# althonos/pyopal

Measured on AMD Instinct MI355X. Metric: GCUPS (billion DP cells/s) SW score-only, 53aa query vs 1Mx300aa DB, higher is better.
Workload: dtype u16; 1 GPU; sw_score q53 (README.md:86) vs 1000000x300 uniform-random proteins per GPU, BLOSUM62, gap_open 3, gap_extend 1; value: blocking miopalSearch, scores in the caller's pinned host array (value_device_results: scores left in HBM); targets_per_gpu=1000000, target_length=300, query_length=53

## Files before the change

include/miopal.h:

```cpp
#ifndef MIOPAL_H
#define MIOPAL_H

#include <stdint.h>

#include "opal.h"

#ifdef __cplusplus
extern "C" {
#endif

typedef struct MiopalDb MiopalDb;

int miopalDeviceCount(void);

const char* miopalLastError(void);

int miopalDbCreate(MiopalDb** out, const unsigned char* const* sequences, const int* lengths,
                   int64_t count, int alphabetLength, int device);

int miopalDbCreateFlat(MiopalDb** out, const unsigned char* residues, const int64_t* offsets,
                       int64_t count, int alphabetLength, int device);

int miopalDbCreateSubset(MiopalDb** out, const MiopalDb* parent, const int64_t* indices, int64_t count);

// ... 23 lines not shown
                         int gapExt, const int* scoreMatrix, int alphabetLength, int searchType,
                         int mode, int64_t start, int64_t end, int* score, int* endTarget,
                         int* endQuery, int* startTarget, int* startQuery,
                         unsigned char** operations, int64_t* operationsCapacity,
                         int64_t* operationOffsets);

int miopalSearchDeviceScores(MiopalDb* db, const unsigned char* query, int queryLength,
                             int gapOpen, int gapExt, const int* scoreMatrix,
                             int alphabetLength, int mode, int64_t start, int64_t end,
                             int* deviceScores, void* stream);

void miopalSetProfiling(MiopalDb* db, int enabled);
int miopalLastKernelTime(MiopalDb* db, float* ms);

void miopalLastRouting(int64_t counts[4]);

int miopalSearchBatch(MiopalDb* db, const unsigned char* queries, const int64_t* queryOffsets, int nQueries,
                      int gapOpen, int gapExt, const int* scoreMatrix, int alphabetLength, int searchType,
                      int mode, int64_t start, int64_t end, int* score, int* endTarget, int* endQuery);

#define MIOPAL_MAX_TOP 4096
int miopalSearchTop(MiopalDb* db, const unsigned char* query, int queryLength, int gapOpen, int gapExt,
                    const int* scoreMatrix, int alphabetLength, int searchType, int mode,
                    int64_t start, int64_t end, int k, int minScore,
                    int* count, int64_t* targetIndex, int* score, int* endTarget, int* endQuery);

int miopalSearchBatchTop(MiopalDb* db, const unsigned char* queries, const int64_t* queryOffsets, int nQueries,
                         int gapOpen, int gapExt, const int* scoreMatrix, int alphabetLength, int searchType,
                         int mode, int64_t start, int64_t end, int k, int minScore,
                         int* count, int64_t* targetIndex, int* score, int* endTarget, int* endQuery);
// ... 35 lines not shown
```

pyopal_amd/_capi.py:

```python

from __future__ import annotations

import ctypes
import os
import typing

import numpy as np

_HERE = os.path.dirname(os.path.abspath(__file__))
LIB_PATH = os.environ.get("MIOPAL_LIBRARY") or os.path.join(_HERE, "libmiopal.so")

OPAL_ERR_OVERFLOW = 1
OPAL_ERR_NO_SIMD_SUPPORT = 2
OPAL_ERR_INVALID_MODE = 3
MIOPAL_MAX_TOP = 4096

SEARCH = {"score": 0, "end": 1, "full": 2}
MODE = {"nw": 0, "hw": 1, "ov": 2, "sw": 3}
OVERFLOW = {"simple": 0, "buckets": 1}


class OpalSearchResult(ctypes.Structure):
    _fields_ = [
        ("scoreSet", ctypes.c_int),
# ... 4 lines not shown
        ("startLocationQuery", ctypes.c_int),
        ("alignment", ctypes.POINTER(ctypes.c_ubyte)),
        ("alignmentLength", ctypes.c_int),
    ]


_lib = None
_libc = None

EXPORTS = [
    "opalInitSearchResult", "opalSearchResultIsEmpty", "opalSearchResultSetScore",
    "opalSearchDatabase", "opalSearchDatabaseCharSW",
    "miopalDeviceCount", "miopalLastError", "miopalDbCreate", "miopalDbCreateFlat", "miopalDbCreateSubset",
    "miopalDbDestroy", "miopalDbCount", "miopalDbTotalLength", "miopalDbDeviceBytes",
    "miopalSearch", "miopalSearchFlat", "miopalSearchFlatInto", "miopalSearchDeviceScores", "miopalSetProfiling", "miopalLastKernelTime",
    "miopalLastRouting", "miopalLastFullRouting", "miopalSearchResults", "miopalReleaseCaches",
    "miopalSearchBatch", "miopalLastBatchRouting", "miopalSearchTop", "miopalSearchBatchTop",
    "miopalAlignPairs", "miopalLastPairRouting",
    "miopalSetTuning", "miopalGetTuning", "miopalDbSetOption", "miopalDbReleaseWorkspaces",
    "miopalSelfTest", "miopalTestInjectFault", "miopalTestSetLogicalDevices",
]


def _share_hip_runtime() -> None:
    import importlib.util
    try:
        spec = importlib.util.find_spec("torch")
    except (ImportError, ValueError):
        spec = None
    if spec is None or not spec.submodule_search_locations:
        return
# ... 64 lines not shown
                                       c_i64, c_i64, c_vp, c_vp, c_vp, c_vp, c_vp,
                                       ctypes.POINTER(c_vp), c_vp]
        L.miopalSearchFlatInto.restype = c_int
        L.miopalSearchFlatInto.argtypes = [c_vp, c_vp, c_int, c_int, c_int, c_vp, c_int, c_int, c_int,
                                           c_i64, c_i64, c_vp, c_vp, c_vp, c_vp, c_vp,
                                           ctypes.POINTER(c_vp), ctypes.POINTER(c_i64), c_vp]
        L.miopalSearchDeviceScores.restype = c_int
        L.miopalSearchDeviceScores.argtypes = [c_vp, c_vp, c_int, c_int, c_int, c_vp, c_int, c_int,
                                               c_i64, c_i64, c_vp, c_vp]
        L.miopalSetProfiling.restype = None
        L.miopalSetProfiling.argtypes = [c_vp, c_int]
        L.miopalReleaseCaches.restype = None
        L.miopalReleaseCaches.argtypes = []
        L.miopalLastFullRouting.restype = c_int
        L.miopalLastFullRouting.argtypes = []
        L.miopalLastRouting.restype = None
        L.miopalLastRouting.argtypes = [ctypes.POINTER(ctypes.c_int64)]
        L.miopalLastKernelTime.restype = c_int
        L.miopalLastKernelTime.argtypes = [c_vp, ctypes.POINTER(ctypes.c_float)]
        L.miopalSearchResults.restype = c_int
        L.miopalSearchResults.argtypes = [c_vp, c_vp, c_int, c_int, c_int, c_vp, c_int, c_vp, c_int,
                                          c_int, c_int, c_i64, c_i64]
        L.opalSearchDatabase.restype = c_int
        L.opalSearchDatabase.argtypes = [c_vp, c_int, c_vp, c_int, c_vp, c_int, c_int, c_vp, c_int,
                                         c_vp, c_int, c_int, c_int]
        _lib = L
        _libc = ctypes.CDLL(None)
        _libc.free.argtypes = [c_vp]
        _libc.free.restype = None
    return _lib
# ... 343 lines not shown
        end = self.count if end is None else min(end, self.count)
        q = np.ascontiguousarray(query, dtype=np.uint8)
        S = np.ascontiguousarray(matrix, dtype=np.int32)
        rc = lib().miopalSearchDeviceScores(self._h, _ptr(q), len(q), gap_open, gap_extend, _ptr(S),
                                            self.alphabet_length, MODE[algorithm], start, end,
                                            ctypes.c_void_p(device_ptr), ctypes.c_void_p(stream))
        raise_for(rc)

    @staticmethod
    def last_routing() -> typing.Tuple[int, int, int, int]:
        counts = (ctypes.c_int64 * 4)()
        lib().miopalLastRouting(counts)
        return tuple(int(c) for c in counts)

    @staticmethod
    def last_full_routing() -> int:
        return int(lib().miopalLastFullRouting())

    def set_profiling(self, enabled: bool) -> None:
        lib().miopalSetProfiling(self._h, 1 if enabled else 0)

    def last_kernel_time(self) -> typing.Tuple[int, float]:
        ms = ctypes.c_float(0)
        n = lib().miopalLastKernelTime(self._h, ctypes.byref(ms))
        return int(n), float(ms.value)
```

pyopal_amd/csrc/common.h:

```cpp
#pragma once
#include <hip/hip_runtime.h>
#include <stdint.h>

namespace miopal {

constexpr int kLanes = 64;
constexpr int kGroupTargets = 128;
constexpr int kMaxAlphabet = 32;
constexpr int kMaxStripRows = 64;

enum Region : int { kLastCell = 0, kLastRow = 1, kLastRowCol = 2, kAllCells = 3 };
struct DpRules {
    int topGap;
    int leftGap;
    int floor0;
    int region;
};

struct InterseqArgs {
    const uint2* pack;
    const int64_t* groupOff;
    const int* groupChunks;
    int nGroups;
    int groupBase;
// ... 22 lines not shown
    int tailThrottle;
    unsigned long long* stripKeys;
    int* stripAbort;
    int stripAbortAt;
    int* stripGaveUp;
    int batchGroups;
    const int32_t* known;
    int32_t* directOut;
    int32_t* directEndI;
    int32_t* directEndJ;
    const int32_t* directIds;
    int directN;
    int stripSpinCap;
    int faultUnit1;
    unsigned long long* stripTiming;
    uint2* boundary[2];
    const int64_t* boundaryOff;
};

struct BatchArgs {
    const uint2* pack;
    const int64_t* groupOff;
    const int* groupChunks;
    const int32_t* lens;
    const int32_t* ids;
    int nPacked;
    int64_t sliceStart;
    const int16_t* profiles;
    int nSymbols;
    const int* qLens;
    const int* qRows;
    int nQueries;
    int unitsPerQuery;
// ... 303 lines not shown
```

pyopal_amd/csrc/host.hip:

```cpp
#include <algorithm>
#include <atomic>
#include <chrono>
#include <condition_variable>
#if defined(__x86_64__)
#include <immintrin.h>
#endif
#include <cstdarg>
#include <cstdio>
#include <cstdlib>
#include <cstring>
#include <deque>
#include <functional>
#include <exception>
#include <ctime>
#include <list>
#include <map>
#include <memory>
#include <mutex>
#include <new>
#include <numeric>
#include <string>
#include <sys/mman.h>
#include <thread>
#include <vector>
// ... 31 lines not shown
        for (int k = 0; k < (int)Tune::kCount; ++k)
            if (strcmp(kTuningNames[k] + 7, name) == 0) return k;
        return -1;
    }
};
}
const char* tuned(Tune key) { return Tuning::table().value[(int)key].load(std::memory_order_acquire); }
}

namespace {

thread_local std::string g_lastError;
thread_local int64_t g_lastRouting[4] = {0, 0, 0, 0};
thread_local int64_t g_lastBatchRouting[4] = {0, 0, 0, 0};
thread_local int g_lastFullRouting = 0;
thread_local int g_fault[3] = {0, 0, 0};
std::atomic<int> g_logicalDevices{0};

const std::vector<int>& usableDevices() {
    static const std::vector<int> list = [] {
        std::vector<int> v;
        int n = 0;
        if (hipGetDeviceCount(&n) != hipSuccess) return v;
        for (int d = 0; d < n; ++d) {
            hipDeviceProp_t p;
            if (hipGetDeviceProperties(&p, d) == hipSuccess && strncmp(p.gcnArchName, "gfx950", 6) == 0) v.push_back(d);
        }
        return v;
    }();
    return list;
// ... 442 lines not shown
        waiter.join();
        if (rcWaiter != 0) return 4;
        if (db->views.size() != 1 || db->views.front().building) return 5;
        db->views.clear();
        return 0;
    });
}

void miopalLastRouting(int64_t counts[4]) {
    if (!counts) return;
    for (int k = 0; k < 4; ++k) counts[k] = g_lastRouting[k];
}

int miopalLastFullRouting(void) { return g_lastFullRouting; }

void miopalLastBatchRouting(int64_t counts[4]) {
    if (!counts) return;
    for (int k = 0; k < 4; ++k) counts[k] = g_lastBatchRouting[k];
}

int miopalLastKernelTime(MiopalDb* db, float* ms) {
    if (!db || !ms) return 0;
    std::lock_guard<std::mutex> g(db->timingMutex);
    *ms = 0.f;
    Workspace* ws = db->lastTimed;
    if (!ws) return 0;
    int n = 0;
    for (auto& ev : ws->timings) {
        float t = 0.f;
        if (hipEventSynchronize(ev.second) == hipSuccess &&
// ... 370 lines not shown
```

pyopal_amd/csrc/host_search.inc:

```
static inline int reservedCus(const MiopalDb* db) {
    const int opt = db->optReserveCus.load(std::memory_order_relaxed);
    if (opt >= 0) return opt;
    if (const char* r = tuned(Tune::RESERVE_CUS)) return std::max(0, atoi(r));
    return -1;
}
static inline bool smallSearchAllowed(const MiopalDb* db) {
    const int opt = db->optSmallSearch.load(std::memory_order_relaxed);
    if (opt >= 0) return opt != 0;
    return !tuned(Tune::NO_SMALL_SEARCH);
}

struct Search {
    MiopalDb* db;
    Workspace* ws;
    hipStream_t stream;
    const unsigned char* query;
    int Q, open, ext, A, searchType, mode;
    const int* matrix;
    int64_t start, end;
    int64_t n;
    int maxScore = 0, minScore = 0;
    int64_t balancedChunks = 0;
    bool globalPairRefused = false;
    bool pairStripsRefused = false;
// ... 190 lines not shown
    }

    int scorePass(int32_t* d_score, int32_t* d_endI, int32_t* d_endJ) {
        return scorePassImpl(d_score, d_endI, d_endJ, true);
    }

    int scorePassImpl(int32_t* d_score, int32_t* d_endI, int32_t* d_endJ, bool useHalf) {
        DpRules r;
        RC_TRY(rulesFor(mode, &r));
        const int rules = packRules(r);
        std::vector<PairJob> jobs;
        RC_TRY(checkInt32(db->maxLen));
        wroteHost = false;

        g_lastRouting[0] = g_lastRouting[1] = g_lastRouting[2] = g_lastRouting[3] = 0;
        bool small = Q <= kLanes && n <= kSmallSearch;
        if (Q > kLanes && n <= kSmallSearch) {
            const int64_t strips = ((int64_t)Q + kLanes - 1) / kLanes;
            const int64_t residues = db->offsets[(size_t)end] - db->offsets[(size_t)start];
            const int64_t steps = strips * (residues + (int64_t)(kLanes - 1) * n);
            if (const char* asked = tuned(Tune::SMALL_STEPS)) {
                small = steps <= atoll(asked);
            } else {
                const double perPair = 0.075 + std::max((double)steps / 7e6, (double)(db->maxLen + kLanes * strips) * 0.00025);
                const double packed = 0.26 + 0.0006 * (double)Q + (Q <= 512 ? 0.0003 * (double)db->maxLen : 0.0);
                small = perPair < packed;
            }
        }
        if (!interseqUsable() || (small && smallSearchAllowed(db))) {
            g_lastRouting[0] = n;
// ... 394 lines not shown
                sideForked = true;
                spt.mark("    side jobs enqueued");
                return 0;
            };
            if (!sideJobs.empty() && !tuned(Tune::NO_SIDE_STREAM)) {
                RC_TRY(ws->ensureAux());
                RC_TRY(ensurePairInputs());
                HIP_TRY(hipEventRecord(ws->evFork, stream));
                HIP_TRY(hipStreamWaitEvent(ws->aux, ws->evFork, 0));
                forked = true;
                sidePending = true;
                besidePersistent = pairStrips;
                if (!tuned(Tune::PACKED_FIRST)) RC_TRY(enqueueSide());
            }
            void *pp, *vs, *vo, *ct;
            RC_TRY(ws->get(kProfile, prof.size() * sizeof(int16_t), &pp));
            RC_TRY(ws->get(kViewScore, (size_t)view->nGroups * kGroupTargets * sizeof(int32_t), &vs));
            RC_TRY(ws->get(kViewOvf, (size_t)view->nGroups * kGroupTargets, &vo));
            RC_TRY(ws->get(kCounter, sizeof(int32_t), &ct));
            RC_TRY(ws->stageUpload(pp, prof.data(), prof.size() * sizeof(prof[0]), stream));
            const int64_t reach = std::min<int64_t>((int64_t)std::min(Q, view->maxPackedLen) * std::max(maxScore, 0), queryBest);
            const int64_t limit = (biased || pairStrips) ? biasedLimit : swShifted ? swLimit : halfFloat ? 2048 : 32767;
            const bool mayOverflow = sw ? (reach >= limit || pairStrips) : globalStrips;
            const int64_t directLimit = tuned(Tune::FIXED_DIRECT_LIMIT) ? kMaxDirectRecompute
                                        : std::max<int64_t>(kMaxDirectRecompute, (view->nPacked - packedSkip) / 8);
            if (mayOverflow) HIP_TRY(hipMemsetAsync(ct, 0, sizeof(int32_t), stream));
            InterseqArgs ia{};
            ia.pack = view->d_pack;
            ia.groupOff = view->d_groupOff;
            ia.groupChunks = view->d_groupChunks;
            ia.nGroups = view->nGroups - firstGroup;
            ia.groupBase = firstGroup;
            ia.profile = (const int16_t*)pp;
            ia.nSymbols = nSym;
            ia.qPad = qPad;
// ... 140 lines not shown
                }
                if (pe != hipSuccess) {
                    (void)hipGetLastError();
                    (globalStrips ? globalStripsRefused : pairStripsRefused) = true;
                    if (tuned(Tune::VERBOSE))
                        fprintf(stderr, "miopal: multi-strip pair-table kernel refused (%s), using the general kernel\n",
                                hipGetErrorString(pe));
                    return scorePassImpl(d_score, d_endI, d_endJ, useHalf);
                }
                if (globalStrips && locate)
                    HIP_TRY(launchDecodeGlobalKeys(ia.stripKeys, view->d_lens, view->nGroups * kGroupTargets, Q, ia.score,
                                                   ia.endI, ia.endJ, stream));
                else if (locate)
                    HIP_TRY(launchDecodeStripKeys(ia.stripKeys, view->nGroups * kGroupTargets, ia.score, ia.endI, ia.endJ, stream));
            } else if (usePair || globalPair) {
                void* wc;
                RC_TRY(ws->get(kWorkCounter, sizeof(int), &wc));
                HIP_TRY(hipMemsetAsync(wc, 0, sizeof(int), stream));
                ia.workCounter = (int*)wc;
                int pairUnits = db->computeUnits;
                if (const int keep = reservedCus(db); keep >= 0)
                    pairUnits = std::max(1, pairUnits - keep);
                else if (forked)
                    pairUnits = std::max(1, pairUnits - (int)std::min<int64_t>(pairUnits / 4, std::max<int64_t>(8, (g_lastRouting[0] + 255) / 256)));
                {
                    const int blocks = std::max(1, std::min(pairUnits, ia.nGroups));
                    const int longest = view->groupChunksHost[firstGroup];
                    const int shortest = view->groupChunksHost[view->nGroups - 1];
                    const char* tt = tuned(Tune::TAIL_THROTTLE);
                    const bool uniform = (int64_t)shortest * 5 >= (int64_t)longest * 4;
                    ia.tailThrottle = (tt ? tt[0] == '1' : uniform) ? (ia.nGroups + blocks * 4 - 1) / (blocks * 4) : 0;
                }
                if ((biased || globalPair) && !mayOverflow && overlap == 0 && !forked && sideJobs.empty() && jobs.empty() &&
                    firstGroup == 0 && packedSkip == 0 && !tuned(Tune::NO_DIRECT_SCATTER)) {
                    int32_t *target = d_score, *targetI = d_endI, *targetJ = d_endJ;
                    if (hostScoreOut && (hostScoreIsCallers || hostScoreGeneration == ws->stagingGeneration) &&
                        (!locate || (hostEndIOut && hostEndJOut)) && !tuned(Tune::NO_HOST_SCATTER)) {
                        target = hostScoreOut;
                        targetI = hostEndIOut;
                        targetJ = hostEndJOut;
                        wroteHost = true;
                    }
                    ia.directOut = target - start;
                    if (locate) {
                        ia.directEndI = targetI - start;
                        ia.directEndJ = targetJ - start;
// ... 114 lines not shown
```

pyopal_amd/csrc/host_workspace.inc:

```
enum Slot {
    kQuery, kMatrix, kProfile, kViewScore, kViewOvf, kCounter, kBoundary0, kBoundary1,
    kScore, kEndI, kEndJ, kJobs, kPairB0, kPairB1, kAuxJobs, kAuxPairB0, kAuxPairB1, kRScore, kRI, kRJ, kDirs, kOps, kOpsOff,
    kOpsLen, kOvfHost, kWorkCounter, kViewEndI, kViewEndJ, kStartQ, kStartT, kMismatch, kCompactOps, kTraceScore, kOpsTotals, kSortBins, kSortedJobs, kScanOrder, kKeys, kHeadWaves, kHeadDirs, kUnitState, kUnitPartial, kStripKeys,
    kPairStripState, kPairStripPartial, kPairStripSpare, kAuxPairStripState, kAuxPairStripPartial, kPairStripError, kStripTiming,
    kBatchProfiles, kBatchMeta, kBatchOverflow,
    kPairListQ, kPairListT, kPairListTOff, kPairListQBase, kPairListQOff, kPairListBoundary,
    kTopScratch,
    kSlots
};

namespace unpack {
#if defined(__x86_64__)
__attribute__((target("bmi2"))) inline void pieces(uint8_t* dst, const uint8_t* packed, int64_t n8) {
    for (int64_t k = 0; k < n8; ++k) {
        uint16_t w;
        memcpy(&w, packed + 2 * k, 2);
        const uint64_t v = __builtin_ia32_pdep_di((uint64_t)w, 0x0303030303030303ull);
        memcpy(dst + 8 * k, &v, 8);
    }
}
inline bool havePdep() {
    static const bool yes = __builtin_cpu_supports("bmi2");
    return yes;
}
// ... 228 lines not shown
    void* buf[kSlots] = {};
    size_t cap[kSlots] = {};
    uint64_t usedBy[kSlots] = {};
    uint64_t leaseStamp = 0;
    std::mutex busy;
    std::vector<std::pair<hipEvent_t, hipEvent_t>> timings;
    hipStream_t aux = nullptr;
    hipEvent_t evFork = nullptr, evJoin = nullptr;

    void* pinned = nullptr;
    size_t pinnedCap = 0, pinnedUsed = 0;
    uint64_t stagingGeneration = 0;
    struct Pending { void* dst; size_t off, bytes; bool onAux = false; };
    std::vector<Pending> pending;
    std::vector<int32_t> hostScratchA, hostScratchB;

    static void copyOut(void* dst, const char* src, size_t bytes) {
        constexpr size_t kPiece = 4u << 20;
        if (bytes < 2 * kPiece) {
            unpack::copyLarge(dst, src, bytes);
            return;
        }
        const int nThreads = (int)std::min<size_t>(4, bytes / kPiece);
        const size_t share = ((bytes / nThreads) + 4095) & ~(size_t)4095;
        std::vector<std::thread> pool;
        for (int t = 1; t < nThreads; ++t) {
            const size_t lo = share * t, hi = std::min(bytes, lo + share);
            if (lo >= hi) continue;
            try {
                pool.emplace_back([=] { unpack::copyLarge((char*)dst + lo, src + lo, hi - lo); });
// ... 100 lines not shown
        HIP_TRY(hipMemcpyAsync((char*)pinned + pinnedUsed, deviceSrc, bytes, hipMemcpyDeviceToHost, onAux ? aux : stream));
        pending.push_back({dst, pinnedUsed, bytes, onAux});
        pinnedUsed += aligned;
        return 0;
    }
    int stageUpload(void* deviceDst, const void* src, size_t bytes, hipStream_t on) {
        if (bytes == 0) return 0;
        const size_t aligned = (bytes + 255) & ~(size_t)255;
        RC_TRY(reserveStaging(aligned));
        memcpy((char*)pinned + pinnedUsed, src, bytes);
        HIP_TRY(hipMemcpyAsync(deviceDst, (const char*)pinned + pinnedUsed, bytes, hipMemcpyHostToDevice, on));
        pinnedUsed += aligned;
        return 0;
    }

    int ensureAux() {
        if (aux) return 0;
        int least = 0, greatest = 0;
        if (hipDeviceGetStreamPriorityRange(&least, &greatest) != hipSuccess) {
            (void)hipGetLastError();
            least = greatest = 0;
        }
        if (greatest != least) HIP_TRY(hipStreamCreateWithPriority(&aux, hipStreamNonBlocking, greatest));
        else HIP_TRY(hipStreamCreateWithFlags(&aux, hipStreamNonBlocking));
        HIP_TRY(hipEventCreateWithFlags(&evFork, hipEventDisableTiming));
        HIP_TRY(hipEventCreateWithFlags(&evJoin, hipEventDisableTiming));
        return 0;
    }

    int get(int slot, size_t bytes, void** out) {
        if (bytes == 0) bytes = 16;
        usedBy[slot] = leaseStamp;
        if (cap[slot] < bytes) {
            if (buf[slot]) {
                HIP_TRY(hipStreamSynchronize(stream));
                HIP_TRY(hipFree(buf[slot]));
                buf[slot] = nullptr;
                cap[slot] = 0;
            }
            size_t want = bytes + bytes / 8 + 256;
            HIP_TRY(hipMalloc(&buf[slot], want));
            cap[slot] = want;
            if (want > (512u << 20) && tuned(Tune::VERBOSE))
                fprintf(stderr, "miopal: workspace slot %d grows to %zu MiB\n", slot, want >> 20);
        }
        *out = buf[slot];
        return 0;
    }
    bool tryGet(int slot, size_t bytes, void** out) {
        usedBy[slot] = leaseStamp;
        if (cap[slot] >= bytes) {
            *out = buf[slot];
            return true;
        }
        if (buf[slot]) {
            (void)hipStreamSynchronize(stream);
            (void)hipFree(buf[slot]);
            buf[slot] = nullptr;
            cap[slot] = 0;
        }
        if (hipMalloc(&buf[slot], bytes) != hipSuccess) {
            (void)hipGetLastError();
            buf[slot] = nullptr;
            return false;
        }
        cap[slot] = bytes;
        if (bytes > (512u << 20) && tuned(Tune::VERBOSE))
            fprintf(stderr, "miopal: workspace slot %d grows to %zu MiB\n", slot, bytes >> 20);
        *out = buf[slot];
        return true;
    }
    size_t bytes() const {
        size_t t = 0;
        for (size_t c : cap) t += c;
        return t;
    }
    size_t trimTo(size_t keep, bool staleOnly = false) {
        size_t freed = 0;
        for (int pass = 0; pass < (staleOnly ? 1 : 2); ++pass)
        while (bytes() > keep) {
            int big = -1;
// ... 26 lines not shown
```

pyopal_amd/csrc/interseq_impl.h:

```cpp
#pragma once
#include <algorithm>

#include <type_traits>

#include "common.h"

namespace miopal {

typedef short s16x2 __attribute__((ext_vector_type(2)));
typedef unsigned short u16x2 __attribute__((ext_vector_type(2)));
typedef _Float16 f16x2 __attribute__((ext_vector_type(2)));

static __device__ __forceinline__ uint32_t pk_add_sat_i16(uint32_t a, uint32_t b) {
    s16x2 r = __builtin_elementwise_add_sat(__builtin_bit_cast(s16x2, a), __builtin_bit_cast(s16x2, b));
    return __builtin_bit_cast(uint32_t, r);
}
static __device__ __forceinline__ uint32_t pk_sub_sat_i16(uint32_t a, uint32_t b) {
    s16x2 r = __builtin_elementwise_sub_sat(__builtin_bit_cast(s16x2, a), __builtin_bit_cast(s16x2, b));
    return __builtin_bit_cast(uint32_t, r);
}
static __device__ __forceinline__ uint32_t pk_max_i16(uint32_t a, uint32_t b) {
    s16x2 r = __builtin_elementwise_max(__builtin_bit_cast(s16x2, a), __builtin_bit_cast(s16x2, b));
    return __builtin_bit_cast(uint32_t, r);
}
// ... 952 lines not shown
        if (lane == 0) *mine = c;
        const int4 p = *simdRow;
        const int behind = __builtin_amdgcn_readfirstlane(min(min(p.x, p.y), min(p.z, p.w)));
        if (c <= behind) __builtin_amdgcn_s_setprio(2);
        else __builtin_amdgcn_s_setprio(0);
    }
};

#ifndef MIOPAL_HEADLINE_PACE
#define MIOPAL_HEADLINE_PACE 1
#endif
#ifndef MIOPAL_HEADLINE_TIMING
#define MIOPAL_HEADLINE_TIMING 0
#endif

template <int R, bool LOC>
__global__ __launch_bounds__(kPairWaves * kLanes) void interseq_pair_biased_kernel(InterseqArgs a) {
    constexpr int SLOTS = PairLayout<R>::kRowSlots;
    constexpr int NB4 = (R + 3) / 4;
    constexpr int kBits = LOC ? locRowBits(R) : 0;
    constexpr int kRowMask = (1 << kBits) - 1;
    extern __shared__ uint4 pairs[];
#if MIOPAL_HEADLINE_TIMING
    const unsigned long long born = __builtin_amdgcn_s_memrealtime();
#endif

    const int lane = threadIdx.x & 63;
    const int nSym = a.nSymbols;
    const int ext = a.gapExt << kBits;
    const uint32_t ext2 = both(ext), openMinusExt2 = both((a.gapOpen << kBits) - ext);
// ... 13 lines not shown
            pw[row * (SLOTS * 4) + r] = (uint32_t)(sB * 65536 + sA);
        }
    }
    int* simdTaken = reinterpret_cast<int*>(pairs + nSym * nSym * SLOTS);
    if (threadIdx.x < 4) simdTaken[threadIdx.x] = 0;
    __syncthreads();
    SimdPace pace;
    if (MIOPAL_HEADLINE_PACE) pace.init(simdTaken + 4, lane);

    const int wave = __builtin_amdgcn_readfirstlane((int)(threadIdx.x >> 6));
    constexpr int kTier[4][3] = {{0, 6, 11}, {1, 7, 8}, {2, 5, 9}, {3, 4, 10}};
    const int tier = kTier[wave & 3][wave >> 2];
    const int firstDynamic = kPairWaves * gridDim.x;
    const int simd = (int)__builtin_amdgcn_s_getreg(4 | (4 << 6) | ((2 - 1) << 11)) & 3;
    bool firstRound = true;
    for (;;) {
        int g;
        if (firstRound) {
            g = tier * gridDim.x + ((tier & 1) ? (int)(gridDim.x - 1 - blockIdx.x) : (int)blockIdx.x);
            firstRound = false;
            if (lane == 0 && a.tailThrottle > 0) atomicAdd(&simdTaken[simd], 1);
            if (g >= a.nGroups) continue;
            g += a.groupBase;
        } else {
            g = 0;
            if (lane == 0) {
                bool take = true;
                if (a.tailThrottle > 0) take = atomicAdd(&simdTaken[simd], 1) < a.tailThrottle;
                g = take ? atomicAdd(a.workCounter, 1) : INT32_MAX - firstDynamic;
            }
            g = __builtin_amdgcn_readfirstlane(g) + firstDynamic;
            if (g >= a.nGroups) break;
            g += a.groupBase;
        }
        const uint2* pack = a.pack + a.groupOff[g];
        const int nChunks = a.groupChunks[g];
        if (nChunks > a.priorityChunks) __builtin_amdgcn_s_setprio(3);
        else __builtin_amdgcn_s_setprio(0);
        uint32_t best = 0u;
        int colA = -1, colB = -1;
        uint32_t fl = zero2 - ext2;
        int shift = -ext;
        uint32_t H[R], E[R];
#pragma unroll
        for (int r = 0; r < R; ++r) {
            H[r] = fl;
            E[r] = zero2;
        }
        uint2 cur = pack[lane];
        auto rowOf = [&](uint32_t tA, uint32_t tB) -> const uint4* {
            const uint32_t rowIdx = __umul24(tA, (uint32_t)nSym) + tB;
            return reinterpret_cast<const uint4*>(reinterpret_cast<const char*>(pairs) +
                                                  __umul24(rowIdx, (uint32_t)(SLOTS * 16)));
        };
#ifndef MIOPAL_PAIR_AHEAD
#define MIOPAL_PAIR_AHEAD 3
#endif
#ifndef MIOPAL_PAIR_XCOL
#define MIOPAL_PAIR_XCOL 1
#endif
        constexpr int kWant = LOC ? (R > 62 ? 1 : R > 58 ? 2 : MIOPAL_PAIR_AHEAD) : (R > 60 ? 2 : MIOPAL_PAIR_AHEAD);
        constexpr int kAhead = NB4 > kWant ? kWant : 1;
        constexpr bool kAcross = MIOPAL_PAIR_XCOL != 0;
        const uint4* prowNext = rowOf(cur.x & 0xffu, cur.y & 0xffu);
        uint4 vn[kAhead];
        if (kAcross) {
#pragma unroll
            for (int k = 0; k < kAhead; ++k) vn[k] = prowNext[k];
        }
        for (int c = 0; c < nChunks; ++c) {
            uint2 nxt = {0, 0};
            if (c + 1 < nChunks) nxt = pack[(size_t)(c + 1) * kLanes + lane];
            if (MIOPAL_HEADLINE_PACE) pace.step(c - nChunks, lane, nChunks > a.priorityChunks);
            uint32_t ra = cur.x, rb = cur.y;
#pragma unroll 1
            for (int cc = 0; cc < 4; ++cc) {
                const uint4* prow = prowNext;
                uint4 v[NB4];
#pragma unroll
                for (int k = 0; k < kAhead; ++k) v[k] = kAcross ? vn[k] : prow[k];
                ra = cc < 3 ? ra >> 8 : nxt.x;
                rb = cc < 3 ? rb >> 8 : nxt.y;
                prowNext = rowOf(ra & 0xffu, rb & 0xffu);
                auto score = [&](int r) -> uint32_t {
                    const uint4 x = v[r >> 2];
// ... 48 lines not shown
                }
            }
            cur = nxt;
            shift += 4 * ext;
            if (shift + 4 * ext > kBiasedMaxShift) {
                const uint32_t d = both(shift);
#pragma unroll
                for (int r = 0; r < R; ++r) {
                    H[r] -= d;
                    E[r] -= d;
                }
                fl -= d;
                shift = 0;
            }
        }
        const int lo = (int)(best & 0xffffu) >> kBits, hi = (int)(best >> 16) >> kBits;
        const size_t base = (size_t)g * kGroupTargets;
        if (a.directOut) {
            const int posA = (int)base + lane, posB = posA + kLanes;
            if (posA < a.directN) {
                const int id = a.directIds[posA];
                a.directOut[id] = lo;
                if constexpr (LOC) {
                    a.directEndI[id] = colA < 0 ? -1 : kRowMask - (int)(best & kRowMask);
                    a.directEndJ[id] = colA;
                }
            }
            if (posB < a.directN) {
                const int id = a.directIds[posB];
                a.directOut[id] = hi;
// ... 1105 lines not shown
```

pyopal_amd/csrc/tuning.h:

```cpp
#pragma once
#include <atomic>

namespace miopal {

#define MIOPAL_TUNING_SWITCHES(X)                                                                          \
    X(ALWAYS_SKIP) X(BATCH_GROUPS) X(DEVICE) X(FIXED_DIRECT_LIMIT) X(FORCE_LANE_PER_PAIR) X(HOST_THREADS)  \
    X(HOST_TRACEBACK) X(LOOSE_REACH) X(NO_BIASED) X(NO_CALLER_PINNED) X(NO_DEFERRED_RESULTS)               \
    X(NO_DIAG_SHIFT) X(NO_DIRECT_SCATTER) X(NO_GLOBAL_STRIPS) X(NO_HOST_SCATTER) X(NO_HUGEPAGE)            \
    X(NO_HYBRID_TRACE) X(NO_OPS_OVERLAP) X(NO_PAIR_STRIPS) X(NO_PAIR_STRIP_UNITS) X(NO_PAIR_TABLE)         \
    X(NO_PERPAIR) X(NO_PERPAIR_PROFILE) X(NO_PRIORITY) X(NO_SCAN_REFILL) X(NO_SEGMENTS) X(NO_SIDE_STREAM)  \
    X(NO_SKIM) X(NO_SMALL_SEARCH) X(NO_SW_SHIFT) X(NO_TWO_PASS_ENDS) X(NO_UNSIGNED_DIAG)                   \
    X(NO_VIEW_PREFETCH) X(PACKED_FIRST) X(PAIR_STRIPS) X(PHASE_TIMING) X(RESERVE_CUS) X(RUNTIME_COPY)      \
    X(SCAN_BLOCKS_PER_CU) X(SCAN_REFILL_LANES) X(SHORT_STRIDE) X(SMALL_STEPS) X(SPARE_HANDLE_MB)           \
    X(STRIPS) X(STRIPS_RESERVE) X(TAIL_THROTTLE) X(THIN_SIDE) X(TWO_PASS_ENDS) X(UNITS)                    \
    X(UPLOAD_PIECE_KB) X(UPLOAD_STREAMS) X(UPLOAD_THREADS) X(VERBOSE) X(VIEW_CACHE_MB)                     \
    X(WINDOWS_WHENEVER_POSSIBLE) X(TEST_REFUSE_PAIR_LAUNCH) X(NO_PACKED_OPS) X(STRIP_TIMING) X(SKIP_SHARES) X(SEARCH_UNDER_UPLOAD) X(NO_WIDE_PAIRS) X(NO_SIDE_COPIES) X(NO_EARLY_HOST_SHARE) X(NO_UNPACK_CREW) X(NO_STREAM_STORES) X(NO_PACKED_TRACE) X(NO_PACKED_SCAN) X(NO_ONE_LAUNCH) X(ONE_LAUNCH_GROUP) X(NO_ASYNC_SHARES) X(NO_LATE_RESULT_COPIES) X(PARKED_WORKSPACE_MB) X(NO_SORT_BY_ROWS) X(NO_JOBS_AHEAD) X(NO_SCAN_ORDER) X(NO_PACKED_HW_SCAN)

enum class Tune : int {
#define X(name) name,
    MIOPAL_TUNING_SWITCHES(X)
#undef X
    kCount
};

const char* tuned(Tune key);

}
```

Before: 10640 GCUPS.

## Add mailbox work handover for tail-idle waves and zero work counter via profile upload

Adds an opt-in handover protocol to the biased pair kernel. Waves that run out of groups park on a ticket in a device mailbox, and busy waves can donate their mid-target DP state (H, E, best, shift) through a mailbox slot so the idle wave finishes the remaining chunks. The aim is to cut tail imbalance at the end of the persistent launch. Separately, the work counter now sits in a zeroed header placed in front of the uploaded profile, which removes a separate memset. The handover path is enabled only through the HANDOVER tuning switch, but the extra kernel code and atomics could affect register use even when it is off.

After: 10590 GCUPS. No clear change (-0.4%).

```diff
diff --git a/include/miopal.h b/include/miopal.h
--- a/include/miopal.h
+++ b/include/miopal.h
@@ -61,6 +61,7 @@
 int miopalLastKernelTime(MiopalDb* db, float* ms);
 
 void miopalLastRouting(int64_t counts[4]);
+int64_t miopalLastHandovers(void);
 
 int miopalSearchBatch(MiopalDb* db, const unsigned char* queries, const int64_t* queryOffsets, int nQueries,
                       int gapOpen, int gapExt, const int* scoreMatrix, int alphabetLength, int searchType,
diff --git a/pyopal_amd/_capi.py b/pyopal_amd/_capi.py
--- a/pyopal_amd/_capi.py
+++ b/pyopal_amd/_capi.py
@@ -42,7 +42,7 @@
     "miopalDeviceCount", "miopalLastError", "miopalDbCreate", "miopalDbCreateFlat", "miopalDbCreateSubset",
     "miopalDbDestroy", "miopalDbCount", "miopalDbTotalLength", "miopalDbDeviceBytes",
     "miopalSearch", "miopalSearchFlat", "miopalSearchFlatInto", "miopalSearchDeviceScores", "miopalSetProfiling", "miopalLastKernelTime",
-    "miopalLastRouting", "miopalLastFullRouting", "miopalSearchResults", "miopalReleaseCaches",
+    "miopalLastRouting", "miopalLastFullRouting", "miopalLastHandovers", "miopalSearchResults", "miopalReleaseCaches",
     "miopalSearchBatch", "miopalLastBatchRouting", "miopalSearchTop", "miopalSearchBatchTop",
     "miopalAlignPairs", "miopalLastPairRouting",
     "miopalSetTuning", "miopalGetTuning", "miopalDbSetOption", "miopalDbReleaseWorkspaces",
@@ -137,6 +137,8 @@
         L.miopalReleaseCaches.argtypes = []
         L.miopalLastFullRouting.restype = c_int
         L.miopalLastFullRouting.argtypes = []
+        L.miopalLastHandovers.restype = c_i64
+        L.miopalLastHandovers.argtypes = []
         L.miopalLastRouting.restype = None
         L.miopalLastRouting.argtypes = [ctypes.POINTER(ctypes.c_int64)]
         L.miopalLastKernelTime.restype = c_int
@@ -510,6 +512,10 @@
         return tuple(int(c) for c in counts)
 
     @staticmethod
+    def last_handovers() -> int:
+        return int(lib().miopalLastHandovers())
+
+    @staticmethod
     def last_full_routing() -> int:
         return int(lib().miopalLastFullRouting())
 
diff --git a/pyopal_amd/csrc/common.h b/pyopal_amd/csrc/common.h
--- a/pyopal_amd/csrc/common.h
+++ b/pyopal_amd/csrc/common.h
@@ -60,9 +60,18 @@
     int stripSpinCap;
     int faultUnit1;
     unsigned long long* stripTiming;
+    int* mailbox;
+    uint32_t* mailTicketWords;
+    int mailTickets, mailSlots;
+    int mailSeq;
+    int handoverMin;
+    int handoverCost;
+    int* handoverCount;
     uint2* boundary[2];
     const int64_t* boundaryOff;
 };
+
+constexpr int kLaunchHeaderBytes = 256;
 
 struct BatchArgs {
     const uint2* pack;
diff --git a/pyopal_amd/csrc/host.hip b/pyopal_amd/csrc/host.hip
--- a/pyopal_amd/csrc/host.hip
+++ b/pyopal_amd/csrc/host.hip
@@ -69,6 +69,20 @@
 thread_local int64_t g_lastRouting[4] = {0, 0, 0, 0};
 thread_local int64_t g_lastBatchRouting[4] = {0, 0, 0, 0};
 thread_local int g_lastFullRouting = 0;
+thread_local const int* g_lastHandoverWord = nullptr;
+static int* handoverWordFor(uint64_t workspaceNumber) {
+    constexpr int kWords = 1024;
+    static int* words = [] {
+        void* p = nullptr;
+        if (hipHostMalloc(&p, kWords * sizeof(int), hipHostMallocDefault) != hipSuccess) {
+            (void)hipGetLastError();
+            return (int*)nullptr;
+        }
+        memset(p, 0, kWords * sizeof(int));
+        return (int*)p;
+    }();
+    return words ? words + workspaceNumber % kWords : nullptr;
+}
 thread_local int g_fault[3] = {0, 0, 0};
 std::atomic<int> g_logicalDevices{0};
 
@@ -541,6 +555,11 @@
 
 int miopalLastFullRouting(void) { return g_lastFullRouting; }
 
+int64_t miopalLastHandovers(void) {
+    const int* word = g_lastHandoverWord;
+    return word ? (int64_t)__atomic_load_n(word, __ATOMIC_ACQUIRE) : 0;
+}
+
 void miopalLastBatchRouting(int64_t counts[4]) {
     if (!counts) return;
     for (int k = 0; k < 4; ++k) counts[k] = g_lastBatchRouting[k];
diff --git a/pyopal_amd/csrc/host_search.inc b/pyopal_amd/csrc/host_search.inc
--- a/pyopal_amd/csrc/host_search.inc
+++ b/pyopal_amd/csrc/host_search.inc
@@ -228,6 +228,7 @@
         wroteHost = false;
 
         g_lastRouting[0] = g_lastRouting[1] = g_lastRouting[2] = g_lastRouting[3] = 0;
+        g_lastHandoverWord = nullptr;
         bool small = Q <= kLanes && n <= kSmallSearch;
         if (Q > kLanes && n <= kSmallSearch) {
             const int64_t strips = ((int64_t)Q + kLanes - 1) / kLanes;
@@ -652,11 +653,13 @@
                 if (!tuned(Tune::PACKED_FIRST)) RC_TRY(enqueueSide());
             }
             void *pp, *vs, *vo, *ct;
-            RC_TRY(ws->get(kProfile, prof.size() * sizeof(int16_t), &pp));
+            void* launchBlock;
+            RC_TRY(ws->get(kProfile, kLaunchHeaderBytes + prof.size() * sizeof(int16_t), &launchBlock));
+            pp = (char*)launchBlock + kLaunchHeaderBytes;
             RC_TRY(ws->get(kViewScore, (size_t)view->nGroups * kGroupTargets * sizeof(int32_t), &vs));
             RC_TRY(ws->get(kViewOvf, (size_t)view->nGroups * kGroupTargets, &vo));
             RC_TRY(ws->get(kCounter, sizeof(int32_t), &ct));
-            RC_TRY(ws->stageUpload(pp, prof.data(), prof.size() * sizeof(prof[0]), stream));
+            RC_TRY(ws->stageUploadBehindZeros(launchBlock, kLaunchHeaderBytes, prof.data(), prof.size() * sizeof(prof[0]), stream));
             const int64_t reach = std::min<int64_t>((int64_t)std::min(Q, view->maxPackedLen) * std::max(maxScore, 0), queryBest);
             const int64_t limit = (biased || pairStrips) ? biasedLimit : swShifted ? swLimit : halfFloat ? 2048 : 32767;
             const bool mayOverflow = sw ? (reach >= limit || pairStrips) : globalStrips;
@@ -827,10 +830,7 @@
                 else if (locate)
                     HIP_TRY(launchDecodeStripKeys(ia.stripKeys, view->nGroups * kGroupTargets, ia.score, ia.endI, ia.endJ, stream));
             } else if (usePair || globalPair) {
-                void* wc;
-                RC_TRY(ws->get(kWorkCounter, sizeof(int), &wc));
-                HIP_TRY(hipMemsetAsync(wc, 0, sizeof(int), stream));
-                ia.workCounter = (int*)wc;
+                ia.workCounter = (int*)launchBlock;
                 int pairUnits = db->computeUnits;
                 if (const int keep = reservedCus(db); keep >= 0)
                     pairUnits = std::max(1, pairUnits - keep);
@@ -843,6 +843,35 @@
                     const char* tt = tuned(Tune::TAIL_THROTTLE);
                     const bool uniform = (int64_t)shortest * 5 >= (int64_t)longest * 4;
                     ia.tailThrottle = (tt ? tt[0] == '1' : uniform) ? (ia.nGroups + blocks * 4 - 1) / (blocks * 4) : 0;
+                    g_lastHandoverWord = nullptr;
+                    const char* ho = tuned(Tune::HANDOVER);
+                    const bool forceHandover = ho && strcmp(ho, "force") == 0;
+                    constexpr int kWavesPerBlock = 12;
+                    const bool pays = uniform && ia.nGroups > blocks * kWavesPerBlock;
+                    int* countWord = handoverWordFor(ws->number);
+                    if (biased && !globalPair && ia.nGroups >= 1 && countWord && (forceHandover || (pays && ho && ho[0] == '1'))) {
+                        const int tickets = std::min(4096, (blocks * kWavesPerBlock + 63) / 64 * 64);
+                        const int slots = std::min(tickets, 1024);
+                        const size_t slotBytes = (size_t)(2 * pairRows + 4) * kLanes * sizeof(uint32_t);
+                        void* mb;
+                        RC_TRY(ws->get(kMailbox, tickets * sizeof(uint32_t) + slots * slotBytes, &mb));
+                        if (ws->mailboxZeroedAt != ws->allocations[kMailbox]) {
+                            HIP_TRY(hipMemsetAsync(mb, 0, tickets * sizeof(uint32_t) + slots * slotBytes, stream));
+                            ws->mailboxZeroedAt = ws->allocations[kMailbox];
+                        }
+                        ws->mailboxSeq = ws->mailboxSeq % 262143u + 1;
+                        ia.mailbox = (int*)launchBlock;
+                        ia.mailTicketWords = (uint32_t*)mb;
+                        ia.mailTickets = tickets;
+                        ia.mailSlots = slots;
+                        ia.mailSeq = (int)ws->mailboxSeq;
+                        const char* hm = tuned(Tune::HANDOVER_MIN);
+                        const char* hc = tuned(Tune::HANDOVER_COST);
+                        ia.handoverMin = forceHandover ? 0 : std::max(1, hm ? atoi(hm) : 8);
+                        ia.handoverCost = std::max(0, hc ? atoi(hc) : 6);
+                        ia.handoverCount = countWord;
+                        g_lastHandoverWord = countWord;
+                    }
                 }
                 if ((biased || globalPair) && !mayOverflow && overlap == 0 && !forked && sideJobs.empty() && jobs.empty() &&
                     firstGroup == 0 && packedSkip == 0 && !tuned(Tune::NO_DIRECT_SCATTER)) {
diff --git a/pyopal_amd/csrc/host_workspace.inc b/pyopal_amd/csrc/host_workspace.inc
--- a/pyopal_amd/csrc/host_workspace.inc
+++ b/pyopal_amd/csrc/host_workspace.inc
@@ -6,6 +6,7 @@
     kBatchProfiles, kBatchMeta, kBatchOverflow,
     kPairListQ, kPairListT, kPairListTOff, kPairListQBase, kPairListQOff, kPairListBoundary,
     kTopScratch,
+    kMailbox,
     kSlots
 };
 
@@ -266,6 +267,13 @@
     struct Pending { void* dst; size_t off, bytes; bool onAux = false; };
     std::vector<Pending> pending;
     std::vector<int32_t> hostScratchA, hostScratchB;
+    uint64_t mailboxZeroedAt = 0;
+    uint32_t mailboxSeq = 0;
+    uint64_t allocations[kSlots] = {};
+    const uint64_t number = [] {
+        static std::atomic<uint64_t> next{0};
+        return next.fetch_add(1);
+    }();
 
     static void copyOut(void* dst, const char* src, size_t bytes) {
         constexpr size_t kPiece = 4u << 20;
@@ -396,6 +404,16 @@
         return 0;
     }
 
+    int stageUploadBehindZeros(void* deviceDst, size_t zeros, const void* src, size_t bytes, hipStream_t on) {
+        const size_t aligned = (zeros + bytes + 255) & ~(size_t)255;
+        RC_TRY(reserveStaging(aligned));
+        memset((char*)pinned + pinnedUsed, 0, zeros);
+        memcpy((char*)pinned + pinnedUsed + zeros, src, bytes);
+        HIP_TRY(hipMemcpyAsync(deviceDst, (const char*)pinned + pinnedUsed, zeros + bytes, hipMemcpyHostToDevice, on));
+        pinnedUsed += aligned;
+        return 0;
+    }
+
     int ensureAux() {
         if (aux) return 0;
         int least = 0, greatest = 0;
@@ -423,6 +441,7 @@
             size_t want = bytes + bytes / 8 + 256;
             HIP_TRY(hipMalloc(&buf[slot], want));
             cap[slot] = want;
+            ++allocations[slot];
             if (want > (512u << 20) && tuned(Tune::VERBOSE))
                 fprintf(stderr, "miopal: workspace slot %d grows to %zu MiB\n", slot, want >> 20);
         }
@@ -447,6 +466,7 @@
             return false;
         }
         cap[slot] = bytes;
+        ++allocations[slot];
         if (bytes > (512u << 20) && tuned(Tune::VERBOSE))
             fprintf(stderr, "miopal: workspace slot %d grows to %zu MiB\n", slot, bytes >> 20);
         *out = buf[slot];
diff --git a/pyopal_amd/csrc/interseq_impl.h b/pyopal_amd/csrc/interseq_impl.h
--- a/pyopal_amd/csrc/interseq_impl.h
+++ b/pyopal_amd/csrc/interseq_impl.h
@@ -990,6 +990,154 @@
 #define MIOPAL_HEADLINE_TIMING 0
 #endif
 
+static_assert(kLaunchHeaderBytes >= 8 * (int)sizeof(int), "the mailbox header");
+#ifndef MIOPAL_HANDOVER_SLEEP
+#define MIOPAL_HANDOVER_SLEEP 64
+#endif
+template <int R>
+struct Handover {
+    enum : uint32_t { kWaiting = 1, kReady = 2, kGone = 3 };
+    static constexpr int kRows = 2 * R + 4;
+    static __device__ __forceinline__ uint32_t* tickets(const InterseqArgs& a) {
+        return a.mailTicketWords;
+    }
+    static __device__ __forceinline__ uint32_t* slotOf(const InterseqArgs& a, int slot) {
+        return tickets(a) + a.mailTickets + (size_t)slot * (kRows * kLanes);
+    }
+    static __device__ __forceinline__ uint32_t word(const InterseqArgs& a, uint32_t state, int payload) {
+        return ((uint32_t)a.mailSeq << 14) | ((uint32_t)min(max(payload, 0), 4095) << 2) | state;
+    }
+    static __device__ __forceinline__ uint32_t ld(const uint32_t* p) {
+        return __hip_atomic_load(const_cast<uint32_t*>(p), __ATOMIC_RELAXED, __HIP_MEMORY_SCOPE_AGENT);
+    }
+    static __device__ __forceinline__ void st(uint32_t* p, uint32_t v) {
+        __hip_atomic_store(p, v, __ATOMIC_RELAXED, __HIP_MEMORY_SCOPE_AGENT);
+    }
+    static __device__ __forceinline__ int add(int* p, int v) {
+        return __hip_atomic_fetch_add(p, v, __ATOMIC_RELAXED, __HIP_MEMORY_SCOPE_AGENT);
+    }
+    static __device__ __forceinline__ int simdLeft(const int4* row) {
+        if (!MIOPAL_HEADLINE_PACE) return 0;
+        const int4 p = *row;
+        const int left = max(-p.x, 0) + max(-p.y, 0) + max(-p.z, 0) + max(-p.w, 0);
+        return __builtin_amdgcn_readfirstlane(left);
+    }
+    static __device__ __forceinline__ uint32_t hint(const InterseqArgs& a) {
+        return ld(reinterpret_cast<const uint32_t*>(a.mailbox) + 6);
+    }
+    static __device__ __forceinline__ int laneId() {
+        return (int)__builtin_amdgcn_mbcnt_hi(~0u, __builtin_amdgcn_mbcnt_lo(~0u, 0u));
+    }
+    static __device__ __forceinline__ void finished(const InterseqArgs& a) {
+        const int lane = laneId();
+        int f = 0;
+        if (lane == 0) f = add(a.mailbox + 1, 1);
+        if (__builtin_amdgcn_readfirstlane(f) != a.nGroups - 1) return;
+        __builtin_amdgcn_fence(__ATOMIC_SEQ_CST, "agent");
+        const int issued = min(__builtin_amdgcn_readfirstlane((int)ld(reinterpret_cast<uint32_t*>(a.mailbox) + 2)), a.mailTickets);
+        for (int t = lane; t < issued; t += kLanes)
+            __hip_atomic_fetch_or(tickets(a) + t, (uint32_t)kGone, __ATOMIC_RELAXED, __HIP_MEMORY_SCOPE_AGENT);
+        if (lane == 0)
+            __hip_atomic_store(a.handoverCount, (int)ld(reinterpret_cast<uint32_t*>(a.mailbox) + 5), __ATOMIC_RELAXED,
+                               __HIP_MEMORY_SCOPE_SYSTEM);
+    }
+    static __device__ __forceinline__ int wait(const InterseqArgs& a, const int4* simdRow) {
+        const int lane = laneId();
+        if (__builtin_amdgcn_readfirstlane((int)ld(reinterpret_cast<uint32_t*>(a.mailbox) + 7)) < (int)gridDim.x) return -1;
+        int t = 0;
+        if (lane == 0) t = add(a.mailbox + 2, 1);
+        t = __builtin_amdgcn_readfirstlane(t);
+        if (t >= a.mailTickets) return -1;
+        uint32_t* mineAt = tickets(a) + t;
+        int left = simdLeft(simdRow);
+        uint32_t mine = word(a, kWaiting, left);
+        if (lane == 0) {
+            st(mineAt, mine);
+            add(a.mailbox + 6, 1);
+        }
+        __builtin_amdgcn_fence(__ATOMIC_SEQ_CST, "agent");
+        bool leave = __builtin_amdgcn_readfirstlane((int)ld(reinterpret_cast<uint32_t*>(a.mailbox) + 1)) >= a.nGroups;
+        if (leave && lane == 0) st(mineAt, mine | kGone);
+        int slot = -1;
+        while (!leave) {
+            __builtin_amdgcn_s_sleep(MIOPAL_HANDOVER_SLEEP);
+            const uint32_t v = __builtin_amdgcn_readfirstlane(ld(mineAt));
+            if (v != mine) {
+                if ((v & 3u) == kReady) slot = (int)((v >> 2) & 4095u);
+                break;
+            }
+            const int now = simdLeft(simdRow);
+            if (now + 8 <= left || now >= left + 8) {
+                uint32_t next = word(a, kWaiting, now), expect = mine;
+                int ok = 0;
+                if (lane == 0)
+                    ok = __hip_atomic_compare_exchange_strong(mineAt, &expect, next, __ATOMIC_RELAXED, __ATOMIC_RELAXED,
+                                                              __HIP_MEMORY_SCOPE_AGENT);
+                if (__builtin_amdgcn_readfirstlane(ok)) {
+                    mine = next;
+                    left = now;
+                }
+            }
+        }
+        if (lane == 0) add(a.mailbox + 6, -1);
+        if (slot >= 0) __builtin_amdgcn_fence(__ATOMIC_ACQUIRE, "agent");
+        return slot;
+    }
+    template <bool LOC>
+    static __device__ __forceinline__ bool donate(const InterseqArgs& a, const int4* simdRow, int lane, int g, int c, int nChunks,
+                                                   int shift, uint32_t best, int colA, int colB, const uint32_t (&H)[R],
+                                                   const uint32_t (&E)[R]) {
+        const int x = nChunks - c;
+        const bool force = a.handoverMin <= 0;
+        int myLeft = 0;
+        if (!force) {
+            myLeft = simdLeft(simdRow);
+            if (x < a.handoverMin || x + a.handoverCost >= myLeft) return false;
+        }
+        const int issued = min(__builtin_amdgcn_readfirstlane((int)ld(reinterpret_cast<uint32_t*>(a.mailbox) + 2)), a.mailTickets);
+        const int served = min(__builtin_amdgcn_readfirstlane((int)ld(reinterpret_cast<uint32_t*>(a.mailbox) + 3)), issued);
+        const int idx = served + lane;
+        uint32_t v = 0;
+        if (idx < issued) v = ld(tickets(a) + idx);
+        const uint32_t state = (v >> 14) == (uint32_t)a.mailSeq ? (v & 3u) : 0u;
+        const uint64_t over = __builtin_amdgcn_ballot_w64(state == kReady || state == kGone);
+        const int lead = ~over == 0 ? kLanes : __builtin_ctzll(~over);
+        if (lead > 0 && lane == 0)
+            __hip_atomic_fetch_max(a.mailbox + 3, served + lead, __ATOMIC_RELAXED, __HIP_MEMORY_SCOPE_AGENT);
+        const int theirs = (int)((v >> 2) & 4095u);
+        uint64_t fit = __builtin_amdgcn_ballot_w64(state == kWaiting && (force || theirs + x + a.handoverCost < myLeft));
+        if (fit == 0) return false;
+        for (int k = g % __builtin_popcountll(fit); k > 0; --k) fit &= fit - 1;
+        const int pick = __builtin_ctzll(fit);
+        const uint32_t seen = __builtin_amdgcn_readlane(v, pick);
+        int slot = 0;
+        if (lane == 0) slot = add(a.mailbox + 4, 1);
+        slot = __builtin_amdgcn_readfirstlane(slot);
+        if (slot >= a.mailSlots) return false;
+        uint32_t* s = slotOf(a, slot) + lane;
+        st(s + 0 * kLanes, lane == 0 ? (uint32_t)g : lane == 1 ? (uint32_t)c : (uint32_t)shift);
+        st(s + 1 * kLanes, best);
+        if (LOC) {
+            st(s + 2 * kLanes, (uint32_t)colA);
+            st(s + 3 * kLanes, (uint32_t)colB);
+        }
+#pragma unroll
+        for (int r = 0; r < R; ++r) {
+            st(s + (4 + r) * kLanes, H[r]);
+            st(s + (4 + R + r) * kLanes, E[r]);
+        }
+        __builtin_amdgcn_fence(__ATOMIC_RELEASE, "agent");
+        int ok = 0;
+        if (lane == 0) {
+            uint32_t expect = seen;
+            ok = __hip_atomic_compare_exchange_strong(tickets(a) + served + pick, &expect, word(a, kReady, slot), __ATOMIC_RELAXED,
+                                                      __ATOMIC_RELAXED, __HIP_MEMORY_SCOPE_AGENT);
+            if (ok) add(a.mailbox + 5, 1);
+        }
+        return __builtin_amdgcn_readfirstlane(ok) != 0;
+    }
+};
+
 template <int R, bool LOC>
 __global__ __launch_bounds__(kPairWaves * kLanes) void interseq_pair_biased_kernel(InterseqArgs a) {
     constexpr int SLOTS = PairLayout<R>::kRowSlots;
@@ -1033,8 +1181,12 @@
     const int firstDynamic = kPairWaves * gridDim.x;
     const int simd = (int)__builtin_amdgcn_s_getreg(4 | (4 << 6) | ((2 - 1) << 11)) & 3;
     bool firstRound = true;
+    typedef Handover<R> Ho;
+    const bool handover = MIOPAL_HEADLINE_PACE && a.mailbox != nullptr;
+    if (handover && threadIdx.x == 0) Ho::add(a.mailbox + 7, 1);
     for (;;) {
         int g;
+        const uint32_t* taken = nullptr;
         if (firstRound) {
             g = tier * gridDim.x + ((tier & 1) ? (int)(gridDim.x - 1 - blockIdx.x) : (int)blockIdx.x);
             firstRound = false;
@@ -1049,8 +1201,23 @@
                 g = take ? atomicAdd(a.workCounter, 1) : INT32_MAX - firstDynamic;
             }
             g = __builtin_amdgcn_readfirstlane(g) + firstDynamic;
-            if (g >= a.nGroups) break;
-            g += a.groupBase;
+            if (g >= a.nGroups) {
+                if (!handover) break;
+                if (lane == 0) *pace.mine = INT32_MAX;
+                const int slot = Ho::wait(a, pace.simdRow);
+                if (slot < 0) break;
+                taken = Ho::slotOf(a, slot);
+            } else {
+                g += a.groupBase;
+            }
+        }
+        int c0 = 0;
+        int shift = -ext;
+        if (taken) {
+            const uint32_t meta = Ho::ld(taken + lane);
+            g = (int)__builtin_amdgcn_readlane(meta, 0);
+            c0 = (int)__builtin_amdgcn_readlane(meta, 1);
+            shift = (int)__builtin_amdgcn_readlane(meta, 2);
         }
         const uint2* pack = a.pack + a.groupOff[g];
         const int nChunks = a.groupChunks[g];
@@ -1058,15 +1225,29 @@
         else __builtin_amdgcn_s_setprio(0);
         uint32_t best = 0u;
         int colA = -1, colB = -1;
-        uint32_t fl = zero2 - ext2;
-        int shift = -ext;
+        uint32_t fl = zero2 + both(shift);
         uint32_t H[R], E[R];
-#pragma unroll
-        for (int r = 0; r < R; ++r) {
-            H[r] = fl;
-            E[r] = zero2;
-        }
-        uint2 cur = pack[lane];
+        if (taken) {
+            best = Ho::ld(taken + 1 * kLanes + lane);
+            if (LOC) {
+                colA = (int)Ho::ld(taken + 2 * kLanes + lane);
+                colB = (int)Ho::ld(taken + 3 * kLanes + lane);
+            }
+#pragma unroll
+            for (int r = 0; r < R; ++r) {
+                H[r] = Ho::ld(taken + (4 + r) * kLanes + lane);
+                E[r] = Ho::ld(taken + (4 + R + r) * kLanes + lane);
+            }
+        } else {
+#pragma unroll
+            for (int r = 0; r < R; ++r) {
+                H[r] = fl;
+                E[r] = zero2;
+            }
+        }
+        uint2 cur = pack[(size_t)c0 * kLanes + lane];
+        uint32_t waiting = 0;
+        bool donated = false;
         auto rowOf = [&](uint32_t tA, uint32_t tB) -> const uint4* {
             const uint32_t rowIdx = __umul24(tA, (uint32_t)nSym) + tB;
             return reinterpret_cast<const uint4*>(reinterpret_cast<const char*>(pairs) +
@@ -1087,7 +1268,15 @@
 #pragma unroll
             for (int k = 0; k < kAhead; ++k) vn[k] = prowNext[k];
         }
-        for (int c = 0; c < nChunks; ++c) {
+        for (int c = c0; c < nChunks; ++c) {
+            if (handover) {
+                if (__builtin_amdgcn_readfirstlane(waiting) != 0 && c > c0 &&
+                    Ho::template donate<LOC>(a, pace.simdRow, lane, g, c, nChunks, shift, best, colA, colB, H, E)) {
+                    donated = true;
+                    break;
+                }
+                waiting = Ho::hint(a);
+            }
             uint2 nxt = {0, 0};
             if (c + 1 < nChunks) nxt = pack[(size_t)(c + 1) * kLanes + lane];
             if (MIOPAL_HEADLINE_PACE) pace.step(c - nChunks, lane, nChunks > a.priorityChunks);
@@ -1166,6 +1355,8 @@
                 shift = 0;
             }
         }
+        if (donated) break;
+        if (handover) Ho::finished(a);
         const int lo = (int)(best & 0xffffu) >> kBits, hi = (int)(best >> 16) >> kBits;
         const size_t base = (size_t)g * kGroupTargets;
         if (a.directOut) {
diff --git a/pyopal_amd/csrc/tuning.h b/pyopal_amd/csrc/tuning.h
--- a/pyopal_amd/csrc/tuning.h
+++ b/pyopal_amd/csrc/tuning.h
@@ -14,7 +14,7 @@
     X(SCAN_BLOCKS_PER_CU) X(SCAN_REFILL_LANES) X(SHORT_STRIDE) X(SMALL_STEPS) X(SPARE_HANDLE_MB)           \
     X(STRIPS) X(STRIPS_RESERVE) X(TAIL_THROTTLE) X(THIN_SIDE) X(TWO_PASS_ENDS) X(UNITS)                    \
     X(UPLOAD_PIECE_KB) X(UPLOAD_STREAMS) X(UPLOAD_THREADS) X(VERBOSE) X(VIEW_CACHE_MB)                     \
-    X(WINDOWS_WHENEVER_POSSIBLE) X(TEST_REFUSE_PAIR_LAUNCH) X(NO_PACKED_OPS) X(STRIP_TIMING) X(SKIP_SHARES) X(SEARCH_UNDER_UPLOAD) X(NO_WIDE_PAIRS) X(NO_SIDE_COPIES) X(NO_EARLY_HOST_SHARE) X(NO_UNPACK_CREW) X(NO_STREAM_STORES) X(NO_PACKED_TRACE) X(NO_PACKED_SCAN) X(NO_ONE_LAUNCH) X(ONE_LAUNCH_GROUP) X(NO_ASYNC_SHARES) X(NO_LATE_RESULT_COPIES) X(PARKED_WORKSPACE_MB) X(NO_SORT_BY_ROWS) X(NO_JOBS_AHEAD) X(NO_SCAN_ORDER) X(NO_PACKED_HW_SCAN)
+    X(WINDOWS_WHENEVER_POSSIBLE) X(TEST_REFUSE_PAIR_LAUNCH) X(NO_PACKED_OPS) X(STRIP_TIMING) X(SKIP_SHARES) X(SEARCH_UNDER_UPLOAD) X(NO_WIDE_PAIRS) X(NO_SIDE_COPIES) X(NO_EARLY_HOST_SHARE) X(NO_UNPACK_CREW) X(NO_STREAM_STORES) X(NO_PACKED_TRACE) X(NO_PACKED_SCAN) X(NO_ONE_LAUNCH) X(ONE_LAUNCH_GROUP) X(NO_ASYNC_SHARES) X(NO_LATE_RESULT_COPIES) X(PARKED_WORKSPACE_MB) X(NO_SORT_BY_ROWS) X(NO_JOBS_AHEAD) X(NO_SCAN_ORDER) X(NO_PACKED_HW_SCAN) X(HANDOVER) X(HANDOVER_MIN) X(HANDOVER_COST)
 
 enum class Tune : int {
 #define X(name) name,
```
